# rimelabs/lambda-labs_distributed-training-guide

Measured on AMD Instinct MI355X. Metric: tokens/sec/GPU (causal-LM pretrain) at 1/2/4/8 MI355X; FSDP peak-mem, higher is better.
Workload: dtype bf16; 1 GPU; model=meta-llama/Meta-Llama-3-8B, global_batch=16, seq_len=1024, parallelism=dp1-single

## Files before the change

csrc/kernels/flash_attn.hip:

```cpp
#include "flash_attn_plan.h"
#include "rope_common.h"

#include <ATen/hip/HIPGeneratorImpl.h>
#include <ATen/hip/PhiloxUtils.cuh>
#include <ATen/core/DistributionsHelper.h>

#include <climits>
#include <cstdlib>
#include <type_traits>

#include <cmath>

namespace dtg {

namespace fa {

typedef __attribute__((address_space(3))) i16x4 lds_i16x4;

constexpr float kLog2e = 1.4426950408889634f;
constexpr float kLn2 = 0.6931471805599453f;
constexpr float kRescaleThreshold = 8.f;

template <int W>
__device__ __forceinline__ int off(int row, int ch) {
// ... 176 lines not shown
    for (int j = 0; j < 2; ++j) {
      uint32_t w[4];
#pragma unroll
      for (int u = 0; u < 2; ++u) {
        const int base = 4 * (2 * j + u);
        w[2 * u + 0] = (uint32_t)f2bf(acc[d][base + 0] * scale) | ((uint32_t)f2bf(acc[d][base + 1] * scale) << 16);
        w[2 * u + 1] = (uint32_t)f2bf(acc[d][base + 2] * scale) | ((uint32_t)f2bf(acc[d][base + 3] * scale) << 16);
      }
#pragma unroll
      for (int x = 0; x < 2; ++x) {
        const auto r = __builtin_amdgcn_permlane32_swap(w[x], w[2 + x], false, false);
        w[x] = r[0];
        w[2 + x] = r[1];
      }
      if (ok) *reinterpret_cast<uint4*>(row + 32 * d + 16 * j + 8 * h) = make_uint4(w[0], w[1], w[2], w[3]);
    }
  }
}

struct KeyRange {
  int start, len, off;
};
__device__ __forceinline__ KeyRange key_range(const int* kstart, const int* klen, int seq, int s0, int seqlen) {
  if (kstart == nullptr) return KeyRange{s0, seqlen, 0};
  const int n = klen[seq];
  return KeyRange{kstart[seq], n, n - seqlen};
}

struct FwdParams {
  const uint16_t *q, *k, *v;
// ... 198 lines not shown
  const float* lse;
  float* delta;
  uint16_t *dq, *dk, *dv;
  int64_t sdq, sdk, sdv;
  const int* cu;
  int64_t T;
  int hq, hkv;
  float scale, c2;
  const int *kstart, *klen;
  int window;
  float *dk_part, *dv_part;
  int nsplit;
  DropCfg drop;
  const float *rope_cos, *rope_sin;
  const int64_t* rope_pos;
};

template <int ND>
__device__ __forceinline__ void rope_inv_rows(f32x16* acc, const float* cos_t, const float* sin_t, int64_t p) {
  constexpr int HT = ND / 2;
  constexpr int HALF = 16 * ND;
  const int h = (threadIdx.x & 63) >> 5;
  const float* cp = cos_t + p * HALF;
  const float* sp = sin_t + p * HALF;
#pragma unroll
  for (int d = 0; d < HT; ++d) {
#pragma unroll
    for (int g = 0; g < 4; ++g) {
      const int i = 32 * d + 8 * g + 4 * h;
      const float4 c = *reinterpret_cast<const float4*>(cp + i);
      const float4 sn = *reinterpret_cast<const float4*>(sp + i);
      const float cc[4] = {c.x, c.y, c.z, c.w}, ss[4] = {sn.x, sn.y, sn.z, sn.w};
#pragma unroll
      for (int e = 0; e < 4; ++e) {
        const int r = 4 * g + e;
        const float x1 = acc[d][r], x2 = acc[d + HT][r];
        acc[d][r] = x1 * cc[e] + x2 * ss[e];
        acc[d + HT][r] = x2 * cc[e] - x1 * ss[e];
      }
    }
  }
}

template <int D, bool CAUSAL, int OCC, bool WIN = false, bool DROP = false>
__global__ __launch_bounds__(256, OCC) void bwd_dq_kernel(BwdParams P) {
  [[maybe_unused]] const DropCfg dcfg = DROP ? resolve_drop(P.drop) : P.drop;
  constexpr int RB = 2 * D;
  constexpr int TILE = kDqBK * RB;
  constexpr int NC = D / 16;
  constexpr int ND = D / 32;
  extern __shared__ __attribute__((aligned(16))) char smem[];

  const int seq = blockIdx.y, head = grid_head(blockIdx.x, P.hq, P.hkv);
  const int s0 = P.cu[seq];
  const int seqlen = P.cu[seq + 1] - s0;
  const int qb = CAUSAL ? (gridDim.z - 1 - blockIdx.z) : blockIdx.z;
  const int q0 = qb * kDqBQ;
  if (q0 >= seqlen) return;
  const KeyRange kr = key_range(P.kstart, P.klen, seq, s0, seqlen);
// ... 152 lines not shown
      char* nb = smem + (1 - B) * 2 * TILE;
      sk.store(nb);
      sv.store(nb + TILE);
    }
    __syncthreads();
  };
  int t = t_begin;
  for (; t + 1 < ntiles; t += 2) {
    tile_step(t, std::integral_constant<int, 0>{});
    tile_step(t + 1, std::integral_constant<int, 1>{});
  }
  if (t < ntiles) tile_step(t, std::integral_constant<int, 0>{});

  if (P.rope_cos != nullptr) rope_inv_rows<ND>(acc, P.rope_cos, P.rope_sin, P.rope_pos[s0 + min(qrow, seqlen - 1)]);
  store_rows_wide<ND>(acc, P.scale, P.dq + (int64_t)(s0 + min(qrow, seqlen - 1)) * P.sdq + (int64_t)head * D, qok);
}

template <int D, bool CAUSAL, int PF, bool WIN = false, int QB = kKvBQ, bool DROP = false>
__global__ __launch_bounds__(256, D == 128 ? 1 : 2) void bwd_dkdv_kernel(BwdParams P) {
  [[maybe_unused]] const DropCfg dcfg = DROP ? resolve_drop(P.drop) : P.drop;
  static_assert(QB == 32 || QB == 64, "query rows per item");
  constexpr int RB = 2 * D;
  constexpr int NC = D / 16;
  constexpr int ND = D / 32;
  constexpr int SLICE = QB * RB;
  extern __shared__ __attribute__((aligned(16))) char smem[];
  char* qd = smem;
  float* rowc = reinterpret_cast<float*>(qd + 4 * SLICE);

  const int seq = blockIdx.y, kvh = blockIdx.x;
  const int s0 = P.cu[seq];
  const int seqlen = P.cu[seq + 1] - s0;
  const KeyRange kr = key_range(P.kstart, P.klen, seq, s0, seqlen);
// ... 269 lines not shown
      float* pv = P.dv_part + o;
#pragma unroll
      for (int d = 0; d < ND; ++d) {
#pragma unroll
        for (int g = 0; g < 4; ++g) {
          *reinterpret_cast<f32x4*>(pk + 32 * d + 8 * g) = f32x4{dk[d][4 * g], dk[d][4 * g + 1], dk[d][4 * g + 2], dk[d][4 * g + 3]};
          *reinterpret_cast<f32x4*>(pv + 32 * d + 8 * g) = f32x4{dv[d][4 * g], dv[d][4 * g + 1], dv[d][4 * g + 2], dv[d][4 * g + 3]};
        }
      }
    }
    return;
  }
  if (P.rope_cos != nullptr) rope_inv_rows<ND>(dk, P.rope_cos, P.rope_sin, P.rope_pos[krow]);
  store_rows_wide<ND>(dk, P.scale, P.dk + krow * P.sdk + (int64_t)kvh * D, key < klen);
  store_rows_wide<ND>(dv, 1.f, P.dv + krow * P.sdv + (int64_t)kvh * D, key < klen);
}

template <int D>
__global__ __launch_bounds__(256) void bwd_kv_combine_kernel(const float* __restrict__ dk_part,
                                                             const float* __restrict__ dv_part, int nsplit,
                                                             int64_t T, int hkv, float scale, uint16_t* __restrict__ dk,
                                                             int64_t sdk, uint16_t* __restrict__ dv, int64_t sdv) {
  constexpr int V = D / 8;
  const int64_t i = (int64_t)blockIdx.x * blockDim.x + threadIdx.x;
  const int64_t rows = T * hkv;
  if (i >= rows * V) return;
  const int64_t row = i / V;
  const int c = (int)(i % V) * 8;
  const int64_t t = row / hkv;
  const int hh = (int)(row % hkv);
// ... 8 lines not shown
    for (int j = 0; j < 4; ++j) {
      a[j] += k0[j];
      a[4 + j] += k1[j];
      b[j] += v0[j];
      b[4 + j] += v1[j];
    }
  }
#pragma unroll
  for (int j = 0; j < 8; ++j) a[j] *= scale;
  store8(dk + t * sdk + (int64_t)hh * D + c, a);
  store8(dv + t * sdv + (int64_t)hh * D + c, b);
}

}

static int env_int(const char* name, int dflt) {
  const char* e = std::getenv(name);
  return (e != nullptr && e[0] != 0) ? std::atoi(e) : dflt;
}
static fa::Tuning& tuning() {
  static fa::Tuning t{std::max(0, env_int("DTG_FA_KV_SPLIT", 0)), env_int("DTG_FA_KV_QB", 64) == 32 ? 32 : 64,
                      env_int("DTG_FA_OCC", 1) == 2 ? 2 : 1, env_int("DTG_FA_KV_PF", 1) == 2 ? 2 : 1};
  return t;
}
[[maybe_unused]] static const bool kTuningLoaded = (tuning(), true);

std::vector<int64_t> flash_attn_tuning(const at::Tensor& , int64_t kv_split, int64_t kv_qb) {
  fa::Tuning& t = tuning();
  std::vector<int64_t> old{t.kv_split, t.kv_qb};
  if (kv_split >= 0) t.kv_split = (int)kv_split;
// ... 2 lines not shown
  return old;
}

template <typename Params>
static void launch(void (*kernel)(Params), const fa::Plan& pl, size_t lds, hipStream_t st, const Params& P) {
  TORCH_INTERNAL_ASSERT(lds == pl.lds, "flash_attn: launch plan and instantiation disagree");
  if (lds > 65536)
    C10_HIP_CHECK(hipFuncSetAttribute((const void*)kernel, hipFuncAttributeMaxDynamicSharedMemorySize, (int)lds));
  hipLaunchKernelGGL(kernel, dim3(pl.grid.x, pl.grid.y, pl.grid.z), dim3(256), lds, st, P);
  DTG_LAUNCH_CHECK();
}
template <int D, bool C, bool WIN = false, bool DROP = false>
static void fwd_launch(const fa::FwdPlan& pl, const fa::FwdParams& P, hipStream_t st) {
  launch(fa::fwd_kernel<D, C, WIN, DROP>, pl, fa::fwd_lds_bytes(D), st, P);
}
template <int D, bool C, int OCC, bool WIN = false, bool DROP = false>
static void dq_launch(const fa::DqPlan& pl, const fa::BwdParams& P, hipStream_t st) {
  TORCH_INTERNAL_ASSERT(pl.occ == OCC);
  launch(fa::bwd_dq_kernel<D, C, OCC, WIN, DROP>, pl, fa::dq_lds_bytes(D), st, P);
}
template <int D, bool C, int PF, bool WIN = false, int QB = fa::kKvBQ, bool DROP = false>
static void kv_launch(const fa::KvPlan& pl, const fa::BwdParams& P, hipStream_t st) {
  TORCH_INTERNAL_ASSERT(pl.pf == PF && pl.qb == QB);
  launch(fa::bwd_dkdv_kernel<D, C, PF, WIN, QB, DROP>, pl, fa::kv_lds_bytes(D, QB), st, P);
}

template <int D>
static void launch_fwd(const fa::FwdPlan& pl, const fa::FwdParams& P, hipStream_t st) {
  if (pl.var == fa::Variant::DROP)
    pl.causal ? fwd_launch<D, true, false, true>(pl, P, st) : fwd_launch<D, false, false, true>(pl, P, st);
  else if (pl.var == fa::Variant::WIN) fwd_launch<D, true, true>(pl, P, st);
  else pl.causal ? fwd_launch<D, true>(pl, P, st) : fwd_launch<D, false>(pl, P, st);
}
template <int D>
static void launch_bwd_dq(const fa::DqPlan& pl, const fa::BwdParams& P, hipStream_t st) {
  constexpr int kOcc = D == 64 ? 2 : 1;
  if (pl.var == fa::Variant::DROP)
    pl.causal ? dq_launch<D, true, kOcc, false, true>(pl, P, st) : dq_launch<D, false, kOcc, false, true>(pl, P, st);
  else if (pl.var == fa::Variant::WIN) dq_launch<D, true, kOcc, true>(pl, P, st);
  else if (pl.occ == 2) pl.causal ? dq_launch<D, true, 2>(pl, P, st) : dq_launch<D, false, 2>(pl, P, st);
  else pl.causal ? dq_launch<D, true, kOcc>(pl, P, st) : dq_launch<D, false, kOcc>(pl, P, st);
}
template <int D>
static void launch_bwd_dkdv(const fa::KvPlan& pl, fa::BwdParams P, hipStream_t st, const at::TensorOptions& opts) {
  at::Tensor dk_part, dv_part;
  P.nsplit = pl.nsplit;
  if (pl.nsplit > 1) {
    dk_part = at::empty({pl.nsplit, P.T, P.hkv, D}, opts.dtype(at::kFloat));
    dv_part = at::empty({pl.nsplit, P.T, P.hkv, D}, opts.dtype(at::kFloat));
    P.dk_part = dk_part.data_ptr<float>();
    P.dv_part = dv_part.data_ptr<float>();
  }
  if (pl.var == fa::Variant::DROP)
    pl.causal ? kv_launch<D, true, 1, false, 64, true>(pl, P, st) : kv_launch<D, false, 1, false, 64, true>(pl, P, st);
  else if (pl.var == fa::Variant::WIN) kv_launch<D, true, 1, true>(pl, P, st);
  else if (pl.pf == 2) pl.causal ? kv_launch<D, true, 2>(pl, P, st) : kv_launch<D, false, 2>(pl, P, st);
  else if (pl.qb == 64)
    pl.causal ? kv_launch<D, true, 1, false, 64>(pl, P, st) : kv_launch<D, false, 1, false, 64>(pl, P, st);
  else pl.causal ? kv_launch<D, true, 1>(pl, P, st) : kv_launch<D, false, 1>(pl, P, st);
  if (pl.nsplit > 1) {
    const int64_t nv = P.T * P.hkv * (D / 8);
    fa::bwd_kv_combine_kernel<D><<<(nv + 255) / 256, 256, 0, st>>>(P.dk_part, P.dv_part, pl.nsplit, P.T, P.hkv, P.scale,
                                                                  P.dk, P.sdk, P.dv, P.sdv);
    DTG_LAUNCH_CHECK();
    if (P.rope_cos != nullptr) rope_rows_launch(P.dk, P.sdk, P.hkv, D, P.rope_cos, P.rope_sin, P.rope_pos, P.T, true, st);
  }
}

struct AttnOpts {
  const at::Tensor *k_start = nullptr, *k_len = nullptr;
  int64_t max_seqlen_k = -1;
  int64_t window = 0;
  const fa::DropCfg* drop = nullptr;
  const at::Tensor *rope_cos = nullptr, *rope_sin = nullptr, *rope_pos = nullptr;
  at::Tensor* stamps = nullptr;
};

static void check_qkv(const at::Tensor& t, const char* name, int64_t heads, int64_t d) {
  DTG_CHECK_CUDA_BF16(t);
  DTG_CHECK(t.dim() == 3 && t.size(1) == heads && t.size(2) == d && t.stride(2) == 1 &&
                t.stride(1) == d && t.stride(0) % 8 == 0,
            name, " must be [T, H, D] with contiguous heads and 16-B aligned token stride");
}

static void check_inputs(const at::Tensor& q, const at::Tensor& k, const at::Tensor& v, const at::Tensor& cu_seqlens) {
  const int64_t D = q.size(2);
  check_qkv(q, "q", q.size(1), D);
  check_qkv(k, "k", k.size(1), D);
  check_qkv(v, "v", k.size(1), D);
  DTG_CHECK(D == 64 || D == 128, "flash_attn: head_dim must be 64 or 128");
// ... 81 lines not shown
  fa::BwdParams P{bf16_ptr(q), bf16_ptr(k), bf16_ptr(v), bf16_ptr(dout), bf16_ptr(o), q.stride(0), k.stride(0),
                  v.stride(0), lse.data_ptr<float>(), delta.data_ptr<float>(), bf16_mut(dq), bf16_mut(dk),
                  bf16_mut(dv), dq.stride(0), dk.stride(0), dv.stride(0), cu_seqlens.data_ptr<int>(), T, (int)hq,
                  (int)hkv, (float)scale, (float)(scale * fa::kLog2e), nullptr, nullptr, 0};
  const fa::Call c = checked_call(q, hkv, nseq, max_seqlen, causal, op, &P.kstart, &P.klen);
  P.window = fa::window_eff(c);
  if (op.rope_cos != nullptr) {
    P.rope_cos = op.rope_cos->data_ptr<float>();
    P.rope_sin = op.rope_sin->data_ptr<float>();
    P.rope_pos = op.rope_pos->data_ptr<int64_t>();
  }
  if (const char* why = fa::conflict(c)) DTG_CHECK(false, why);
  if (op.drop != nullptr) P.drop = *op.drop;
  const fa::DqPlan dqp = fa::plan_dq(c, tuning());
  const fa::KvPlan kvp = fa::plan_kv(c, tuning());
  D == 128 ? launch_bwd_dq<128>(dqp, P, stream()) : launch_bwd_dq<64>(dqp, P, stream());
  D == 128 ? launch_bwd_dkdv<128>(kvp, P, stream(), q.options()) : launch_bwd_dkdv<64>(kvp, P, stream(), q.options());
}

static std::tuple<at::Tensor, at::Tensor, at::Tensor> flash_attn_bwd_alloc(
    const at::Tensor& dout, const at::Tensor& q, const at::Tensor& k, const at::Tensor& v, const at::Tensor& o,
    const at::Tensor& lse, const at::Tensor& cu_seqlens, int64_t max_seqlen, double scale, bool causal,
    const AttnOpts& op) {
  auto dq = at::empty(q.sizes(), q.options());
  auto dk = op.k_start != nullptr ? at::zeros(k.sizes(), k.options()) : at::empty(k.sizes(), k.options());
  auto dv = op.k_start != nullptr ? at::zeros(v.sizes(), v.options()) : at::empty(v.sizes(), v.options());
  flash_attn_bwd_impl(dout, q, k, v, o, lse, cu_seqlens, max_seqlen, scale, causal, dq, dk, dv, op);
  return {dq, dk, dv};
}

static at::Tensor flash_attn_bwd_fused(const char* name, const at::Tensor& dout, const at::Tensor& qkv, int64_t nq,
                                       int64_t nkv, int64_t D, const at::Tensor& o, const at::Tensor& lse,
                                       const at::Tensor& cu_seqlens, int64_t max_seqlen, double scale, bool causal,
                                       const AttnOpts& op) {
  rope::check_qkv(qkv, nq + 2 * nkv, D, name);
  const int64_t T = qkv.size(0);
  DTG_CHECK(qkv.size(1) == (nq + 2 * nkv) * D, name, ": qkv must be [T, (nq + 2 nkv) * D]");
  if (op.rope_cos != nullptr) {
    rope::check_tables(*op.rope_cos, *op.rope_sin, D, name);
    rope::check_pos(*op.rope_pos, T, name);
  }
  auto dqkv = at::empty({T, (nq + 2 * nkv) * D}, qkv.options());
  auto view3 = [&](const at::Tensor& t, int64_t h0, int64_t nh) {
    return t.as_strided({T, nh, D}, {t.stride(0), D, 1}, t.storage_offset() + h0 * D);
  };
  flash_attn_bwd_impl(dout, view3(qkv, 0, nq), view3(qkv, nq, nkv), view3(qkv, nq + nkv, nkv), o, lse, cu_seqlens,
                      max_seqlen, scale, causal, view3(dqkv, 0, nq), view3(dqkv, nq, nkv), view3(dqkv, nq + nkv, nkv), op);
  return dqkv;
}

std::tuple<at::Tensor, at::Tensor, at::Tensor> flash_attn_bwd(
    const at::Tensor& dout, const at::Tensor& q, const at::Tensor& k, const at::Tensor& v, const at::Tensor& o,
    const at::Tensor& lse, const at::Tensor& cu_seqlens, int64_t max_seqlen, double scale, bool causal, int64_t window) {
  return flash_attn_bwd_alloc(dout, q, k, v, o, lse, cu_seqlens, max_seqlen, scale, causal, {.window = window});
}

at::Tensor flash_attn_bwd_qkv(const at::Tensor& dout, const at::Tensor& qkv, int64_t nq, int64_t nkv, int64_t head_dim,
                              const at::Tensor& o, const at::Tensor& lse, const at::Tensor& cu_seqlens,
                              int64_t max_seqlen, double scale, bool causal, int64_t window) {
  return flash_attn_bwd_fused("flash_attn_bwd_qkv", dout, qkv, nq, nkv, head_dim, o, lse, cu_seqlens, max_seqlen, scale,
                              causal, {.window = window});
}

at::Tensor flash_attn_bwd_qkv_rope(const at::Tensor& dout, const at::Tensor& qkv, int64_t nq, int64_t nkv, int64_t head_dim,
                                   const at::Tensor& o, const at::Tensor& lse, const at::Tensor& cu_seqlens,
                                   int64_t max_seqlen, double scale, bool causal, const at::Tensor& cos_t,
                                   const at::Tensor& sin_t, const at::Tensor& pos, int64_t window) {
  return flash_attn_bwd_fused("flash_attn_bwd_qkv_rope", dout, qkv, nq, nkv, head_dim, o, lse, cu_seqlens, max_seqlen,
                              scale, causal, {.window = window, .rope_cos = &cos_t, .rope_sin = &sin_t, .rope_pos = &pos});
}

std::tuple<at::Tensor, at::Tensor> flash_attn_varlen_fwd(
    const at::Tensor& q, const at::Tensor& k, const at::Tensor& v, const at::Tensor& cu_seqlens_q,
    const at::Tensor& k_start, const at::Tensor& k_len, int64_t max_seqlen_q,
    int64_t , double scale, bool causal) {
  return flash_attn_fwd_impl(q, k, v, cu_seqlens_q, max_seqlen_q, scale, causal, {.k_start = &k_start, .k_len = &k_len});
}

std::tuple<at::Tensor, at::Tensor, at::Tensor> flash_attn_varlen_bwd(
    const at::Tensor& dout, const at::Tensor& q, const at::Tensor& k, const at::Tensor& v, const at::Tensor& o,
    const at::Tensor& lse, const at::Tensor& cu_seqlens_q, const at::Tensor& k_start, const at::Tensor& k_len,
    int64_t max_seqlen_q, int64_t max_seqlen_k, double scale, bool causal) {
  return flash_attn_bwd_alloc(dout, q, k, v, o, lse, cu_seqlens_q, max_seqlen_q, scale, causal,
                              {.k_start = &k_start, .k_len = &k_len, .max_seqlen_k = max_seqlen_k});
// ... 58 lines not shown
  return out;
}

TORCH_LIBRARY_IMPL(dtg, CUDA, m) {
  m.impl("flash_attn_fwd_drop", &flash_attn_fwd_drop);
  m.impl("flash_attn_bwd_drop", &flash_attn_bwd_drop);
  m.impl("flash_attn_bwd_qkv_drop", &flash_attn_bwd_qkv_drop);
  m.impl("philox_rng", &philox_rng);
  m.impl("flash_attn_varlen_fwd", &flash_attn_varlen_fwd);
  m.impl("flash_attn_varlen_bwd", &flash_attn_varlen_bwd);
  m.impl("flash_attn_fwd", &flash_attn_fwd);
  m.impl("flash_attn_fwd_stamped", &flash_attn_fwd_stamped);
  m.impl("flash_attn_bwd", &flash_attn_bwd);
  m.impl("flash_attn_bwd_qkv", &flash_attn_bwd_qkv);
  m.impl("flash_attn_bwd_qkv_rope", &flash_attn_bwd_qkv_rope);
  m.impl("flash_attn_tuning", &flash_attn_tuning);
}

}
```

csrc/kernels/flash_attn_plan.h:

```cpp
#pragma once

#include <algorithm>
#include <cstddef>
#include <cstdint>

namespace dtg {
namespace fa {

constexpr int kFwdBQ = 128;
constexpr int kFwdBK = 64;
constexpr int kDqBQ = 128;
constexpr int kDqBK = 64;
constexpr int kKvBK = 128;
constexpr int kKvBQ = 32;

constexpr size_t fwd_lds_bytes(int D) { return 4 * (size_t)kFwdBK * D * 2; }
constexpr size_t dq_lds_bytes(int D) { return 4 * (size_t)kDqBK * D * 2 + kDqBQ * 4; }
constexpr size_t kv_lds_bytes(int D, int qb) { return 4 * (size_t)qb * D * 2 + 2 * 2 * qb * 4; }

struct Tuning {
  int kv_split, kv_qb, dq_occ, kv_pf;
};
struct Call {
  int D;
// ... 42 lines not shown
}

inline KvPlan plan_kv(const Call& c, const Tuning& t) {
  const Variant var = variant(c);
  const int pf = var == Variant::PLAIN && !c.key_ranges ? t.kv_pf : 1;
  const int qb = c.drop || (t.kv_qb != 32 && window_eff(c) == 0 && t.kv_pf == 1) ? 64 : 32;
  const unsigned nkb = nblocks(c.max_seqlen_k, kKvBK);
  const int64_t wgs = (int64_t)c.hkv * c.nseq * nkb;
  int nsplit = 1;
  if (t.kv_split > 0) nsplit = std::min(8, t.kv_split);
  else if (wgs > 0 && wgs < 512) nsplit = (int)std::min<int64_t>(4, (512 + wgs - 1) / wgs);
  if (c.key_ranges || window_eff(c) != 0 || (c.drop ? 1 : t.kv_pf) != 1) nsplit = 1;
  return {{var, c.causal, {(unsigned)c.hkv, (unsigned)c.nseq, nkb * nsplit}, kv_lds_bytes(c.D, qb)}, pf, qb, nsplit};
}

}
}
```

lambda-labs_distributed-training-guide_amd/models/llama.py:

```python
from __future__ import annotations

import dataclasses
import weakref
from typing import Optional

import torch
import torch.distributed as dist
import torch.nn as nn

from .. import ops
from ..parallel import async_tp, tp_comm
from .config import LlamaConfig


@dataclasses.dataclass
class CausalLMOutput:
    loss: Optional[torch.Tensor] = None
    logits: Optional[torch.Tensor] = None


class Weight(nn.Module):

    _dtg_param_holder = True

# ... 59 lines not shown
            k = qkv[:, self.nq * d:(self.nq + self.nkv) * d].reshape(T, self.nkv, d)
            v = qkv[:, (self.nq + self.nkv) * d:].reshape(T, self.nkv, d)
            return cp_attention(q, k, v, rc.cp_group, rc.rows, ranges=rc.cp_ranges).reshape(T, self.nq * d)
        if rc.sp_group is not None:
            from ..parallel.ulysses import ulysses_attention

            qkv = ops.qk_norm_rope(qkv, wq, wk, self.eps, self.nq, self.nkv, d)
            return ulysses_attention(qkv, self.nq, self.nkv, d, rc.sp_group, rc.rows, rc.cu_seqlens,
                                     rc.max_seqlen, rc.cos, rc.sin, rc.pos)
        qkv = ops.qk_norm_rope(qkv, wq, wk, self.eps, self.nq, self.nkv, d, rc.cos, rc.sin, rc.pos,
                               grad_inplace=True)
        return ops.attention(qkv, self.nq, self.nkv, d, rc.cu_seqlens, rc.max_seqlen, window=self.window)

    def forward(self, x, rc: RunCtx, out=None):
        b = getattr(self.qkv_proj, "bias", None)
        qkv = ops.linear(x, self.qkv_proj.weight, None if b is None else b.view(-1))
        if self.qk_norm:
            return ops.linear(self._forward_qk_norm(qkv, rc), self.o_proj.weight, out=out)
        if rc.cp_group is not None:
            from ..parallel.context_parallel import cp_attention

            T, d = qkv.shape[0], self.d
            qkv = ops.rope(qkv, rc.cos, rc.sin, rc.pos, self.nq + self.nkv, d)
            q = qkv[:, :self.nq * d].reshape(T, self.nq, d)
            k = qkv[:, self.nq * d:(self.nq + self.nkv) * d].reshape(T, self.nkv, d)
            v = qkv[:, (self.nq + self.nkv) * d:].reshape(T, self.nkv, d)
            o = cp_attention(q, k, v, rc.cp_group, rc.rows, ranges=rc.cp_ranges).reshape(T, self.nq * d)
        elif rc.sp_group is not None:
            from ..parallel.ulysses import ulysses_attention

# ... 295 lines not shown
```

lambda-labs_distributed-training-guide_amd/ops/__init__.py:

```python
from . import _schema
from . import _cpu
from . import _native

_native.load()
if not _native.LOADED:
    _schema.LIB.impl("adamw_cpu_", lambda p, g, m, v, lr, b1, b2, eps, wd, step, gs: _cpu.adamw_(
        p, None, g, m, v, lr, b1, b2, eps, wd, step, gs), "CPU")

from .functional import (
    add_rms_norm,
    attention,
    check_sample_scalar,
    decode_attention,
    decode_attention_multi,
    dropout_add_layer_norm,
    embedding,
    fused_linear_cross_entropy,
    gelu_mlp,
    kv_cache_append,
    layer_norm,
    linear,
    qk_norm_rope,
    quantize_fp8_rows,
    rms_norm,
    rope,
    rope_tables,
    sample_logits,
    skinny_linear,
    skinny_linear_fp8,
    swiglu,
    swiglu_mlp,
    vocab_parallel_fused_linear_cross_entropy,
)
from .grad_routing import route_param_grad
from .adamw import adamw_step

import contextlib as _contextlib
# ... 3 lines not shown

@_contextlib.contextmanager
def fa_tuning(device="cuda", kv_split: int = -1, kv_qb: int = -1):
    like = _torch.empty(0, device=device)
    old = _torch.ops.dtg.flash_attn_tuning(like, kv_split, kv_qb)
    try:
        yield
    finally:
        _torch.ops.dtg.flash_attn_tuning(like, old[0], old[1])

__all__ = [
    "add_rms_norm", "attention", "rope", "embedding", "fused_linear_cross_entropy", "linear", "rms_norm",
    "rope_tables", "swiglu", "swiglu_mlp", "vocab_parallel_fused_linear_cross_entropy", "route_param_grad", "adamw_step",
    "fa_tuning", "layer_norm", "dropout_add_layer_norm", "gelu_mlp", "qk_norm_rope", "kv_cache_append", "decode_attention",
    "sample_logits", "skinny_linear", "skinny_linear_fp8", "quantize_fp8_rows", "decode_attention_multi",
]
```

lambda-labs_distributed-training-guide_amd/ops/_cpu.py:

```python
import math

import torch
import torch.nn.functional as F

from ._schema import LIB

_LOG2E = 1.4426950408889634


def rmsnorm_fwd(x, w, eps):
    xf = x.float()
    rstd = torch.rsqrt(xf.pow(2).mean(-1) + eps)
    n = (xf * rstd[:, None]).to(x.dtype)
    y = (w.float() * n.float()).to(x.dtype)
    return y, rstd


def add_rmsnorm_fwd(x, res, w, eps):
    h = (x.float() + res.float()).to(x.dtype)
    y, rstd = rmsnorm_fwd(h, w, eps)
    return y, h, rstd


def rmsnorm_bwd(dy, x, w, rstd, dres):
# ... 674 lines not shown
    q, k, v = _qkv_heads(qkv, nq, nkv, head_dim)
    dq, dk, dv = flash_attn_bwd(dout, q, k, v, o, lse, cu_seqlens, max_seqlen, scale, causal, window)
    return torch.cat([dq.reshape(T, -1), dk.reshape(T, -1), dv.reshape(T, -1)], dim=1)


def flash_attn_bwd_qkv_rope(dout, qkv, nq, nkv, head_dim, o, lse, cu_seqlens, max_seqlen, scale, causal, cos, sin,
                            pos, window=0):
    T = qkv.shape[0]
    q, k, v = _qkv_heads(qkv, nq, nkv, head_dim)
    dq, dk, dv = _flash_attn_bwd_f32(dout, q, k, v, o, lse, cu_seqlens, max_seqlen, scale, causal, window)
    dqkv = torch.cat([dq.reshape(T, -1), dk.reshape(T, -1), dv.reshape(T, -1)], dim=1)
    rope_(dqkv, cos, sin, pos, nq + nkv, head_dim, True)
    return dqkv.to(qkv.dtype)


def swiglu_bwd_t(dh, gu):
    if not (gu.dim() == 2 and gu.stride(1) == 1 and gu.stride(0) % 8 == 0 and gu.shape[1] % 16 == 0):
        raise RuntimeError("dtg: swiglu_bwd_t: the pre-activation must be [T, 2 * I] with unit inner stride, "
                           "16-byte aligned rows and I % 8 == 0")
    if not (dh.dim() == 2 and dh.shape[0] == gu.shape[0] and dh.shape[1] == gu.shape[1] // 2):
        raise RuntimeError("dtg: swiglu_bwd_t: shape mismatch")
    dgu = swiglu_bwd(dh, gu)
    return dgu, dgu.t().contiguous(), swiglu_fwd(gu).t().contiguous()


def transpose2d(x):
    return x.t().contiguous()


def transpose_mats_(x, out, mats, mats_host, ntiles):
# ... 84 lines not shown
def flash_attn_tuning(like, kv_split, kv_qb):
    old = list(_TUNING)
    if kv_split >= 0:
        _TUNING[0] = int(kv_split)
    if kv_qb >= 0:
        _TUNING[1] = int(kv_qb)
    return old


for _name, _fn in list(globals().items()):
    if _name in (
        "rmsnorm_fwd", "add_rmsnorm_fwd", "rmsnorm_bwd", "rope_", "swiglu_fwd", "swiglu_bwd",
        "ce_fwd_bwd_", "ce_stats", "ce_grad_", "adamw_", "adamw_t_", "grad_sumsq_", "flash_attn_fwd", "flash_attn_bwd",
        "flash_attn_bwd_qkv", "transpose2d", "transpose_mats_", "swiglu_bwd_t", "embedding_bwd_", "flash_attn_varlen_fwd",
        "flash_attn_varlen_bwd", "flash_attn_fwd_drop", "flash_attn_bwd_drop", "flash_attn_bwd_qkv_drop", "philox_rng",
        "flash_attn_bwd_qkv_rope", "flash_attn_tuning", "layernorm_fwd", "dropout_add_layernorm_fwd", "layernorm_bwd",
        "gelu_fwd", "gelu_bwd", "gelu_bwd_t", "qk_norm_rope_fwd_", "qk_norm_rope_bwd_", "kv_cache_append_", "decode_attn",
        "sample_logits", "skinny_linear", "skinny_linear_fp8", "decode_attn_multi",
        "kv_cache_append_fp8_", "decode_attn_fp8",
    ):
        LIB.impl(_name, _fn, "CPU")
```

lambda-labs_distributed-training-guide_amd/ops/_schema.py:

```python
import torch

LIB = torch.library.Library("dtg", "DEF")

_DEFS = [
    "rmsnorm_fwd(Tensor x, Tensor w, float eps) -> (Tensor, Tensor)",
    "add_rmsnorm_fwd(Tensor x, Tensor residual, Tensor w, float eps) -> (Tensor, Tensor, Tensor)",
    "rmsnorm_bwd(Tensor dy, Tensor x, Tensor w, Tensor rstd, Tensor? dres) -> (Tensor, Tensor)",
    "layernorm_fwd(Tensor x, Tensor w, Tensor b, float eps) -> (Tensor, Tensor, Tensor)",
    "dropout_add_layernorm_fwd(Tensor x, Tensor residual, Tensor w, Tensor b, float eps, float p, Tensor? rng) "
    "-> (Tensor, Tensor, Tensor, Tensor)",
    "layernorm_bwd(Tensor dy, Tensor h, Tensor w, Tensor mean, Tensor rstd, Tensor? dres, float p, Tensor? rng) "
    "-> (Tensor, Tensor, Tensor, Tensor)",
    "gelu_fwd(Tensor x) -> Tensor",
    "gelu_bwd(Tensor dh, Tensor x) -> Tensor",
    "gelu_bwd_t(Tensor dh, Tensor x) -> (Tensor, Tensor, Tensor)",
    "rope_(Tensor(a!) qkv, Tensor cos, Tensor sin, Tensor pos, int nheads, int head_dim, bool inverse) -> ()",
    "qk_norm_rope_fwd_(Tensor(a!) qkv, Tensor wq, Tensor wk, Tensor cos, Tensor sin, Tensor pos, int nq, int nkv, "
    "int head_dim, float eps) -> (Tensor, Tensor)",
    "qk_norm_rope_bwd_(Tensor(a!) dqkv, Tensor xqk, Tensor rstd, Tensor wq, Tensor wk, Tensor cos, Tensor sin, "
    "Tensor pos, int nq, int nkv, int head_dim) -> (Tensor, Tensor)",
    "kv_cache_append_(Tensor(a!) qkv, Tensor(b!) k_cache, Tensor(c!) v_cache, Tensor cos, Tensor sin, Tensor pos, "
    "Tensor rows, int nq, int nkv, int head_dim) -> ()",
    "decode_attn(Tensor qkv, Tensor k_cache, Tensor v_cache, Tensor rows, Tensor lens, int nq, int nkv, int head_dim, "
    "float scale, int max_len, int window=0, int splits=0) -> Tensor",
# ... 17 lines not shown
    "adamw_t_(Tensor(a!) p, Tensor(b!)? master, Tensor g, Tensor(c!) m, Tensor(d!) v, Tensor(e!) pt, Tensor mats, "
    "int ntiles, float lr, float beta1, float beta2, float eps, float wd, int step, float grad_scale, "
    "Tensor? hyper=None, int tile_cols=64, Tensor? gscale=None) -> ()",
    "grad_sumsq_(Tensor g, Tensor(a!) acc, int slot) -> ()",
    "adamw_cpu_(Tensor(a!) p, Tensor g, Tensor(b!) m, Tensor(c!) v, float lr, float beta1, float beta2, "
    "float eps, float wd, int step, float grad_scale) -> ()",
    "flash_attn_fwd(Tensor q, Tensor k, Tensor v, Tensor cu_seqlens, int max_seqlen, float scale, bool causal, "
    "int window=0) -> (Tensor, Tensor)",
    "flash_attn_bwd(Tensor dout, Tensor q, Tensor k, Tensor v, Tensor o, Tensor lse, Tensor cu_seqlens, "
    "int max_seqlen, float scale, bool causal, int window=0) -> (Tensor, Tensor, Tensor)",
    "flash_attn_bwd_qkv(Tensor dout, Tensor qkv, int nq, int nkv, int head_dim, Tensor o, Tensor lse, "
    "Tensor cu_seqlens, int max_seqlen, float scale, bool causal, int window=0) -> Tensor",
    "flash_attn_bwd_qkv_rope(Tensor dout, Tensor qkv, int nq, int nkv, int head_dim, Tensor o, Tensor lse, "
    "Tensor cu_seqlens, int max_seqlen, float scale, bool causal, Tensor cos, Tensor sin, Tensor pos, "
    "int window=0) -> Tensor",
    "flash_attn_fwd_drop(Tensor q, Tensor k, Tensor v, Tensor cu_seqlens, int max_seqlen, float scale, bool causal, "
    "float p, Tensor rng) -> (Tensor, Tensor)",
    "flash_attn_bwd_drop(Tensor dout, Tensor q, Tensor k, Tensor v, Tensor o, Tensor lse, Tensor cu_seqlens, "
    "int max_seqlen, float scale, bool causal, float p, Tensor rng) -> (Tensor, Tensor, Tensor)",
    "flash_attn_bwd_qkv_drop(Tensor dout, Tensor qkv, int nq, int nkv, int head_dim, Tensor o, Tensor lse, "
    "Tensor cu_seqlens, int max_seqlen, float scale, bool causal, float p, Tensor rng) -> Tensor",
    "philox_rng(Tensor like, int increment) -> Tensor",
    "transpose2d(Tensor x) -> Tensor",
    "transpose_mats_(Tensor x, Tensor(a!) out, Tensor mats, Tensor mats_host, int ntiles) -> ()",
    "embedding_bwd_(Tensor(a!) out, Tensor ids, Tensor dy) -> ()",
    "flash_attn_varlen_fwd(Tensor q, Tensor k, Tensor v, Tensor cu_seqlens_q, Tensor k_start, Tensor k_len, "
    "int max_seqlen_q, int max_seqlen_k, float scale, bool causal) -> (Tensor, Tensor)",
    "flash_attn_varlen_bwd(Tensor dout, Tensor q, Tensor k, Tensor v, Tensor o, Tensor lse, Tensor cu_seqlens_q, "
    "Tensor k_start, Tensor k_len, int max_seqlen_q, int max_seqlen_k, float scale, bool causal) "
    "-> (Tensor, Tensor, Tensor)",
# ... 8 lines not shown
```

lambda-labs_distributed-training-guide_amd/ops/functional.py:

```python
import math
import os

import torch
import torch.distributed as dist
import torch.nn.functional as F

from . import grad_routing as _gr
from ._cpu import SKINNY_MAX_M
from .grad_routing import route_embedding_grad, route_param_grad, route_weight_grad_mm

ops = torch.ops.dtg


_LINEAR_BWD = os.environ.get("DTG_LINEAR_BWD", "tn")
_TN_MIN_TOKENS = 4096


def _tn_ok(*ts):
    return all(t.is_cuda and t.dtype == torch.bfloat16 and t.shape[0] % 8 == 0 and t.shape[1] % 8 == 0
               and t.stride(1) == 1 for t in ts)


def _wt(w):
    ref = getattr(w, "_dtg_wt", None)
# ... 211 lines not shown

    @staticmethod
    def backward(ctx, do):
        qkv, o, lse, cu, cos, sin, pos = ctx.saved_tensors
        max_seqlen, nq, nkv, d, scale, causal, rope, window = ctx.meta
        T = qkv.shape[0]
        if rope and _FA_ROPE_FUSED:
            dqkv = ops.flash_attn_bwd_qkv_rope(do.contiguous().view(T, nq, d), qkv, nq, nkv, d, o, lse, cu, max_seqlen,
                                               scale, causal, cos, sin, pos, window)
        else:
            dqkv = ops.flash_attn_bwd_qkv(do.contiguous().view(T, nq, d), qkv, nq, nkv, d, o, lse, cu, max_seqlen,
                                          scale, causal, window)
            if rope:
                ops.rope_(dqkv, cos, sin, pos, nq + nkv, d, True)
        return dqkv, None, None, None, None, None, None, None, None, None, None, None, None


class _AttentionQKVDrop(torch.autograd.Function):

    @staticmethod
    def forward(ctx, qkv, cu_seqlens, max_seqlen, nq, nkv, head_dim, scale, causal, p, rng):
        T = qkv.shape[0]
        d = head_dim
        q, k, v = _qkv_head_views(qkv, nq, nkv, d)
        o, lse = ops.flash_attn_fwd_drop(q, k, v, cu_seqlens, max_seqlen, scale, causal, p, rng)
        ctx.save_for_backward(qkv, o, lse, cu_seqlens, rng)
        ctx.meta = (max_seqlen, nq, nkv, d, scale, causal, p)
        return o.view(T, nq * d)

    @staticmethod
# ... 695 lines not shown
```

Before: 27740 tokens/s (whole job).

## Fuse QKV projection with attention and emit transposed dQKV from backward kernels

Adds a combined QKV-projection + flash-attention autograd function whose backward asks the flash-attention dq and dkdv kernels to also write a transposed copy of dQKV, scattered column-wise. That copy then feeds the weight-gradient matmul directly. The aim is to drop the separate transpose pass and the extra layout traffic when computing dW in TN layout. The cost is strided, uncoalesced 2-byte column stores from the attention kernels, plus one extra [3D*heads, T] buffer.

```diff
diff --git a/csrc/kernels/flash_attn.hip b/csrc/kernels/flash_attn.hip
--- a/csrc/kernels/flash_attn.hip
+++ b/csrc/kernels/flash_attn.hip
@@ -214,6 +214,20 @@
         w[2 + x] = r[1];
       }
       if (ok) *reinterpret_cast<uint4*>(row + 32 * d + 16 * j + 8 * h) = make_uint4(w[0], w[1], w[2], w[3]);
+    }
+  }
+}
+
+template <int ND>
+__device__ __forceinline__ void store_cols_t(const f32x16* acc, float scale, uint16_t* col0, int64_t T, bool ok) {
+  if (!ok) return;
+  const int h = (threadIdx.x & 63) >> 5;
+#pragma unroll
+  for (int d = 0; d < ND; ++d) {
+#pragma unroll
+    for (int g = 0; g < 4; ++g) {
+#pragma unroll
+      for (int e = 0; e < 4; ++e) col0[(int64_t)(32 * d + 8 * g + 4 * h + e) * T] = f2bf(acc[d][4 * g + e] * scale);
     }
   }
 }
@@ -442,6 +456,7 @@
   DropCfg drop;
   const float *rope_cos, *rope_sin;
   const int64_t* rope_pos;
+  uint16_t *dq_t, *dk_t, *dv_t;
 };
 
 template <int ND>
@@ -470,7 +485,7 @@
   }
 }
 
-template <int D, bool CAUSAL, int OCC, bool WIN = false, bool DROP = false>
+template <int D, bool CAUSAL, int OCC, bool WIN = false, bool DROP = false, bool TR = false>
 __global__ __launch_bounds__(256, OCC) void bwd_dq_kernel(BwdParams P) {
   [[maybe_unused]] const DropCfg dcfg = DROP ? resolve_drop(P.drop) : P.drop;
   constexpr int RB = 2 * D;
@@ -653,9 +668,10 @@
 
   if (P.rope_cos != nullptr) rope_inv_rows<ND>(acc, P.rope_cos, P.rope_sin, P.rope_pos[s0 + min(qrow, seqlen - 1)]);
   store_rows_wide<ND>(acc, P.scale, P.dq + (int64_t)(s0 + min(qrow, seqlen - 1)) * P.sdq + (int64_t)head * D, qok);
-}
-
-template <int D, bool CAUSAL, int PF, bool WIN = false, int QB = kKvBQ, bool DROP = false>
+  if constexpr (TR) store_cols_t<ND>(acc, P.scale, P.dq_t + (int64_t)head * D * P.T + t_row, P.T, qok);
+}
+
+template <int D, bool CAUSAL, int PF, bool WIN = false, int QB = kKvBQ, bool DROP = false, bool TR = false>
 __global__ __launch_bounds__(256, D == 128 ? 1 : 2) void bwd_dkdv_kernel(BwdParams P) {
   [[maybe_unused]] const DropCfg dcfg = DROP ? resolve_drop(P.drop) : P.drop;
   static_assert(QB == 32 || QB == 64, "query rows per item");
@@ -955,6 +971,10 @@
   if (P.rope_cos != nullptr) rope_inv_rows<ND>(dk, P.rope_cos, P.rope_sin, P.rope_pos[krow]);
   store_rows_wide<ND>(dk, P.scale, P.dk + krow * P.sdk + (int64_t)kvh * D, key < klen);
   store_rows_wide<ND>(dv, 1.f, P.dv + krow * P.sdv + (int64_t)kvh * D, key < klen);
+  if constexpr (TR) {
+    store_cols_t<ND>(dk, P.scale, P.dk_t + (int64_t)kvh * D * P.T + krow, P.T, key < klen);
+    store_cols_t<ND>(dv, 1.f, P.dv_t + (int64_t)kvh * D * P.T + krow, P.T, key < klen);
+  }
 }
 
 template <int D>
@@ -993,6 +1013,8 @@
 
 }
 
+at::Tensor transpose2d(const at::Tensor& x);
+
 static int env_int(const char* name, int dflt) {
   const char* e = std::getenv(name);
   return (e != nullptr && e[0] != 0) ? std::atoi(e) : dflt;
@@ -1025,15 +1047,15 @@
 static void fwd_launch(const fa::FwdPlan& pl, const fa::FwdParams& P, hipStream_t st) {
   launch(fa::fwd_kernel<D, C, WIN, DROP>, pl, fa::fwd_lds_bytes(D), st, P);
 }
-template <int D, bool C, int OCC, bool WIN = false, bool DROP = false>
+template <int D, bool C, int OCC, bool WIN = false, bool DROP = false, bool TR = false>
 static void dq_launch(const fa::DqPlan& pl, const fa::BwdParams& P, hipStream_t st) {
-  TORCH_INTERNAL_ASSERT(pl.occ == OCC);
-  launch(fa::bwd_dq_kernel<D, C, OCC, WIN, DROP>, pl, fa::dq_lds_bytes(D), st, P);
-}
-template <int D, bool C, int PF, bool WIN = false, int QB = fa::kKvBQ, bool DROP = false>
+  TORCH_INTERNAL_ASSERT(pl.occ == OCC && TR == (P.dq_t != nullptr));
+  launch(fa::bwd_dq_kernel<D, C, OCC, WIN, DROP, TR>, pl, fa::dq_lds_bytes(D), st, P);
+}
+template <int D, bool C, int PF, bool WIN = false, int QB = fa::kKvBQ, bool DROP = false, bool TR = false>
 static void kv_launch(const fa::KvPlan& pl, const fa::BwdParams& P, hipStream_t st) {
-  TORCH_INTERNAL_ASSERT(pl.pf == PF && pl.qb == QB);
-  launch(fa::bwd_dkdv_kernel<D, C, PF, WIN, QB, DROP>, pl, fa::kv_lds_bytes(D, QB), st, P);
+  TORCH_INTERNAL_ASSERT(pl.pf == PF && pl.qb == QB && TR == (P.dk_t != nullptr));
+  launch(fa::bwd_dkdv_kernel<D, C, PF, WIN, QB, DROP, TR>, pl, fa::kv_lds_bytes(D, QB), st, P);
 }
 
 template <int D>
@@ -1046,7 +1068,11 @@
 template <int D>
 static void launch_bwd_dq(const fa::DqPlan& pl, const fa::BwdParams& P, hipStream_t st) {
   constexpr int kOcc = D == 64 ? 2 : 1;
-  if (pl.var == fa::Variant::DROP)
+  if (P.dq_t != nullptr) {
+    TORCH_INTERNAL_ASSERT(fa::dq_emits_t(pl, D));
+    pl.causal ? dq_launch<D, true, kOcc, false, false, true>(pl, P, st)
+              : dq_launch<D, false, kOcc, false, false, true>(pl, P, st);
+  } else if (pl.var == fa::Variant::DROP)
     pl.causal ? dq_launch<D, true, kOcc, false, true>(pl, P, st) : dq_launch<D, false, kOcc, false, true>(pl, P, st);
   else if (pl.var == fa::Variant::WIN) dq_launch<D, true, kOcc, true>(pl, P, st);
   else if (pl.occ == 2) pl.causal ? dq_launch<D, true, 2>(pl, P, st) : dq_launch<D, false, 2>(pl, P, st);
@@ -1062,7 +1088,11 @@
     P.dk_part = dk_part.data_ptr<float>();
     P.dv_part = dv_part.data_ptr<float>();
   }
-  if (pl.var == fa::Variant::DROP)
+  if (P.dk_t != nullptr) {
+    TORCH_INTERNAL_ASSERT(fa::kv_emits_t(pl));
+    pl.causal ? kv_launch<D, true, 1, false, 64, false, true>(pl, P, st)
+              : kv_launch<D, false, 1, false, 64, false, true>(pl, P, st);
+  } else if (pl.var == fa::Variant::DROP)
     pl.causal ? kv_launch<D, true, 1, false, 64, true>(pl, P, st) : kv_launch<D, false, 1, false, 64, true>(pl, P, st);
   else if (pl.var == fa::Variant::WIN) kv_launch<D, true, 1, true>(pl, P, st);
   else if (pl.pf == 2) pl.causal ? kv_launch<D, true, 2>(pl, P, st) : kv_launch<D, false, 2>(pl, P, st);
@@ -1085,6 +1115,8 @@
   const fa::DropCfg* drop = nullptr;
   const at::Tensor *rope_cos = nullptr, *rope_sin = nullptr, *rope_pos = nullptr;
   at::Tensor* stamps = nullptr;
+  const at::Tensor* dqkv_t = nullptr;
+  bool* dqkv_t_written = nullptr;
 };
 
 static void check_qkv(const at::Tensor& t, const char* name, int64_t heads, int64_t d) {
@@ -1196,6 +1228,12 @@
   if (op.drop != nullptr) P.drop = *op.drop;
   const fa::DqPlan dqp = fa::plan_dq(c, tuning());
   const fa::KvPlan kvp = fa::plan_kv(c, tuning());
+  if (op.dqkv_t != nullptr && op.k_start == nullptr && fa::dq_emits_t(dqp, (int)D) && fa::kv_emits_t(kvp)) {
+    P.dq_t = bf16_mut(*op.dqkv_t);
+    P.dk_t = P.dq_t + hq * D * T;
+    P.dv_t = P.dk_t + hkv * D * T;
+    *op.dqkv_t_written = true;
+  }
   D == 128 ? launch_bwd_dq<128>(dqp, P, stream()) : launch_bwd_dq<64>(dqp, P, stream());
   D == 128 ? launch_bwd_dkdv<128>(kvp, P, stream(), q.options()) : launch_bwd_dkdv<64>(kvp, P, stream(), q.options());
 }
@@ -1214,7 +1252,7 @@
 static at::Tensor flash_attn_bwd_fused(const char* name, const at::Tensor& dout, const at::Tensor& qkv, int64_t nq,
                                        int64_t nkv, int64_t D, const at::Tensor& o, const at::Tensor& lse,
                                        const at::Tensor& cu_seqlens, int64_t max_seqlen, double scale, bool causal,
-                                       const AttnOpts& op) {
+                                       AttnOpts op, at::Tensor* dqkv_t = nullptr) {
   rope::check_qkv(qkv, nq + 2 * nkv, D, name);
   const int64_t T = qkv.size(0);
   DTG_CHECK(qkv.size(1) == (nq + 2 * nkv) * D, name, ": qkv must be [T, (nq + 2 nkv) * D]");
@@ -1223,11 +1261,18 @@
     rope::check_pos(*op.rope_pos, T, name);
   }
   auto dqkv = at::empty({T, (nq + 2 * nkv) * D}, qkv.options());
+  bool t_written = false;
+  if (dqkv_t != nullptr) {
+    *dqkv_t = at::empty({(nq + 2 * nkv) * D, T}, qkv.options());
+    op.dqkv_t = dqkv_t;
+    op.dqkv_t_written = &t_written;
+  }
   auto view3 = [&](const at::Tensor& t, int64_t h0, int64_t nh) {
     return t.as_strided({T, nh, D}, {t.stride(0), D, 1}, t.storage_offset() + h0 * D);
   };
   flash_attn_bwd_impl(dout, view3(qkv, 0, nq), view3(qkv, nq, nkv), view3(qkv, nq + nkv, nkv), o, lse, cu_seqlens,
                       max_seqlen, scale, causal, view3(dqkv, 0, nq), view3(dqkv, nq, nkv), view3(dqkv, nq + nkv, nkv), op);
+  if (dqkv_t != nullptr && !t_written) *dqkv_t = transpose2d(dqkv);
   return dqkv;
 }
 
@@ -1250,6 +1295,26 @@
                                    const at::Tensor& sin_t, const at::Tensor& pos, int64_t window) {
   return flash_attn_bwd_fused("flash_attn_bwd_qkv_rope", dout, qkv, nq, nkv, head_dim, o, lse, cu_seqlens, max_seqlen,
                               scale, causal, {.window = window, .rope_cos = &cos_t, .rope_sin = &sin_t, .rope_pos = &pos});
+}
+
+std::tuple<at::Tensor, at::Tensor> flash_attn_bwd_qkv_t(
+    const at::Tensor& dout, const at::Tensor& qkv, int64_t nq, int64_t nkv, int64_t head_dim, const at::Tensor& o,
+    const at::Tensor& lse, const at::Tensor& cu_seqlens, int64_t max_seqlen, double scale, bool causal,
+    const c10::optional<at::Tensor>& cos_t, const c10::optional<at::Tensor>& sin_t,
+    const c10::optional<at::Tensor>& pos, int64_t window) {
+  const bool rope = cos_t.has_value();
+  DTG_CHECK(rope == sin_t.has_value() && rope == pos.has_value(), "flash_attn_bwd_qkv_t: cos, sin and pos go together");
+  DTG_CHECK(qkv.dim() == 2 && qkv.size(0) % 8 == 0, "flash_attn_bwd_qkv_t: the token count must be a multiple of 8");
+  AttnOpts op{.window = window};
+  if (rope) {
+    op.rope_cos = &*cos_t;
+    op.rope_sin = &*sin_t;
+    op.rope_pos = &*pos;
+  }
+  at::Tensor dqkv_t;
+  auto dqkv = flash_attn_bwd_fused("flash_attn_bwd_qkv_t", dout, qkv, nq, nkv, head_dim, o, lse, cu_seqlens, max_seqlen,
+                                   scale, causal, op, &dqkv_t);
+  return {dqkv, dqkv_t};
 }
 
 std::tuple<at::Tensor, at::Tensor> flash_attn_varlen_fwd(
@@ -1338,6 +1403,7 @@
   m.impl("flash_attn_bwd", &flash_attn_bwd);
   m.impl("flash_attn_bwd_qkv", &flash_attn_bwd_qkv);
   m.impl("flash_attn_bwd_qkv_rope", &flash_attn_bwd_qkv_rope);
+  m.impl("flash_attn_bwd_qkv_t", &flash_attn_bwd_qkv_t);
   m.impl("flash_attn_tuning", &flash_attn_tuning);
 }
 
diff --git a/csrc/kernels/flash_attn_plan.h b/csrc/kernels/flash_attn_plan.h
--- a/csrc/kernels/flash_attn_plan.h
+++ b/csrc/kernels/flash_attn_plan.h
@@ -80,5 +80,8 @@
   return {{var, c.causal, {(unsigned)c.hkv, (unsigned)c.nseq, nkb * nsplit}, kv_lds_bytes(c.D, qb)}, pf, qb, nsplit};
 }
 
+inline bool dq_emits_t(const DqPlan& p, int D) { return p.var == Variant::PLAIN && p.occ == (D == 64 ? 2 : 1); }
+inline bool kv_emits_t(const KvPlan& p) { return p.var == Variant::PLAIN && p.pf == 1 && p.qb == 64 && p.nsplit <= 1; }
+
 }
 }
diff --git a/lambda-labs_distributed-training-guide_amd/models/llama.py b/lambda-labs_distributed-training-guide_amd/models/llama.py
--- a/lambda-labs_distributed-training-guide_amd/models/llama.py
+++ b/lambda-labs_distributed-training-guide_amd/models/llama.py
@@ -97,6 +97,10 @@
 
     def forward(self, x, rc: RunCtx, out=None):
         b = getattr(self.qkv_proj, "bias", None)
+        if b is None and not self.qk_norm and rc.cp_group is None and rc.sp_group is None:
+            o = ops.qkv_attention(x, self.qkv_proj.weight, self.nq, self.nkv, self.d, rc.cu_seqlens, rc.max_seqlen,
+                                  rc.cos, rc.sin, rc.pos, window=self.window)
+            return ops.linear(o, self.o_proj.weight, out=out)
         qkv = ops.linear(x, self.qkv_proj.weight, None if b is None else b.view(-1))
         if self.qk_norm:
             return ops.linear(self._forward_qk_norm(qkv, rc), self.o_proj.weight, out=out)
diff --git a/lambda-labs_distributed-training-guide_amd/ops/__init__.py b/lambda-labs_distributed-training-guide_amd/ops/__init__.py
--- a/lambda-labs_distributed-training-guide_amd/ops/__init__.py
+++ b/lambda-labs_distributed-training-guide_amd/ops/__init__.py
@@ -21,6 +21,7 @@
     layer_norm,
     linear,
     qk_norm_rope,
+    qkv_attention,
     quantize_fp8_rows,
     rms_norm,
     rope,
@@ -54,4 +55,5 @@
     "rope_tables", "swiglu", "swiglu_mlp", "vocab_parallel_fused_linear_cross_entropy", "route_param_grad", "adamw_step",
     "fa_tuning", "layer_norm", "dropout_add_layer_norm", "gelu_mlp", "qk_norm_rope", "kv_cache_append", "decode_attention",
     "sample_logits", "skinny_linear", "skinny_linear_fp8", "quantize_fp8_rows", "decode_attention_multi",
+    "qkv_attention",
 ]
diff --git a/lambda-labs_distributed-training-guide_amd/ops/_cpu.py b/lambda-labs_distributed-training-guide_amd/ops/_cpu.py
--- a/lambda-labs_distributed-training-guide_amd/ops/_cpu.py
+++ b/lambda-labs_distributed-training-guide_amd/ops/_cpu.py
@@ -712,6 +712,20 @@
     return dqkv.to(qkv.dtype)
 
 
+def flash_attn_bwd_qkv_t(dout, qkv, nq, nkv, head_dim, o, lse, cu_seqlens, max_seqlen, scale, causal, cos, sin, pos,
+                         window=0):
+    if (cos is None) != (sin is None) or (cos is None) != (pos is None):
+        raise RuntimeError("dtg: flash_attn_bwd_qkv_t: cos, sin and pos go together")
+    if qkv.shape[0] % 8:
+        raise RuntimeError("dtg: flash_attn_bwd_qkv_t: the token count must be a multiple of 8")
+    if cos is None:
+        dqkv = flash_attn_bwd_qkv(dout, qkv, nq, nkv, head_dim, o, lse, cu_seqlens, max_seqlen, scale, causal, window)
+    else:
+        dqkv = flash_attn_bwd_qkv_rope(dout, qkv, nq, nkv, head_dim, o, lse, cu_seqlens, max_seqlen, scale, causal, cos,
+                                       sin, pos, window)
+    return dqkv, dqkv.t().contiguous()
+
+
 def swiglu_bwd_t(dh, gu):
     if not (gu.dim() == 2 and gu.stride(1) == 1 and gu.stride(0) % 8 == 0 and gu.shape[1] % 16 == 0):
         raise RuntimeError("dtg: swiglu_bwd_t: the pre-activation must be [T, 2 * I] with unit inner stride, "
@@ -826,7 +840,7 @@
         "ce_fwd_bwd_", "ce_stats", "ce_grad_", "adamw_", "adamw_t_", "grad_sumsq_", "flash_attn_fwd", "flash_attn_bwd",
         "flash_attn_bwd_qkv", "transpose2d", "transpose_mats_", "swiglu_bwd_t", "embedding_bwd_", "flash_attn_varlen_fwd",
         "flash_attn_varlen_bwd", "flash_attn_fwd_drop", "flash_attn_bwd_drop", "flash_attn_bwd_qkv_drop", "philox_rng",
-        "flash_attn_bwd_qkv_rope", "flash_attn_tuning", "layernorm_fwd", "dropout_add_layernorm_fwd", "layernorm_bwd",
+        "flash_attn_bwd_qkv_rope", "flash_attn_bwd_qkv_t", "flash_attn_tuning", "layernorm_fwd", "dropout_add_layernorm_fwd", "layernorm_bwd",
         "gelu_fwd", "gelu_bwd", "gelu_bwd_t", "qk_norm_rope_fwd_", "qk_norm_rope_bwd_", "kv_cache_append_", "decode_attn",
         "sample_logits", "skinny_linear", "skinny_linear_fp8", "decode_attn_multi",
         "kv_cache_append_fp8_", "decode_attn_fp8",
diff --git a/lambda-labs_distributed-training-guide_amd/ops/_schema.py b/lambda-labs_distributed-training-guide_amd/ops/_schema.py
--- a/lambda-labs_distributed-training-guide_amd/ops/_schema.py
+++ b/lambda-labs_distributed-training-guide_amd/ops/_schema.py
@@ -55,6 +55,9 @@
     "flash_attn_bwd_qkv_rope(Tensor dout, Tensor qkv, int nq, int nkv, int head_dim, Tensor o, Tensor lse, "
     "Tensor cu_seqlens, int max_seqlen, float scale, bool causal, Tensor cos, Tensor sin, Tensor pos, "
     "int window=0) -> Tensor",
+    "flash_attn_bwd_qkv_t(Tensor dout, Tensor qkv, int nq, int nkv, int head_dim, Tensor o, Tensor lse, "
+    "Tensor cu_seqlens, int max_seqlen, float scale, bool causal, Tensor? cos, Tensor? sin, Tensor? pos, "
+    "int window=0) -> (Tensor, Tensor)",
     "flash_attn_fwd_drop(Tensor q, Tensor k, Tensor v, Tensor cu_seqlens, int max_seqlen, float scale, bool causal, "
     "float p, Tensor rng) -> (Tensor, Tensor)",
     "flash_attn_bwd_drop(Tensor dout, Tensor q, Tensor k, Tensor v, Tensor o, Tensor lse, Tensor cu_seqlens, "
diff --git a/lambda-labs_distributed-training-guide_amd/ops/functional.py b/lambda-labs_distributed-training-guide_amd/ops/functional.py
--- a/lambda-labs_distributed-training-guide_amd/ops/functional.py
+++ b/lambda-labs_distributed-training-guide_amd/ops/functional.py
@@ -249,6 +249,63 @@
             if rope:
                 ops.rope_(dqkv, cos, sin, pos, nq + nkv, d, True)
         return dqkv, None, None, None, None, None, None, None, None, None, None, None, None
+
+
+_FUSED_T = os.environ.get("DTG_FUSED_T", "1") == "1"
+
+
+class _QKVAttention(torch.autograd.Function):
+
+    @staticmethod
+    def forward(ctx, x, w, cos, sin, pos, cu_seqlens, max_seqlen, nq, nkv, head_dim, scale, causal, rope, window):
+        T, d = x.shape[0], head_dim
+        qkv = torch.mm(x, w.t())
+        if rope:
+            ops.rope_(qkv, cos, sin, pos, nq + nkv, d, False)
+        q, k, v = _qkv_head_views(qkv, nq, nkv, d)
+        o, lse = ops.flash_attn_fwd(q, k, v, cu_seqlens, max_seqlen, scale, causal, window)
+        ctx.save_for_backward(x, w, qkv, o, lse, cu_seqlens, cos, sin, pos)
+        ctx.meta = (max_seqlen, nq, nkv, d, scale, causal, rope, window)
+        return o.view(T, nq * d)
+
+    @staticmethod
+    def backward(ctx, do):
+        x, w, qkv, o, lse, cu, cos, sin, pos = ctx.saved_tensors
+        max_seqlen, nq, nkv, d, scale, causal, rope, window = ctx.meta
+        T = qkv.shape[0]
+        dx_tn, dw_tn = _bwd_layout(x, w)
+        do = do.contiguous().view(T, nq, d)
+        fused_rope = rope and _FA_ROPE_FUSED
+        dqkv_t = None
+        if _FUSED_T and dw_tn and ctx.needs_input_grad[1] and _tn_ok(qkv) and (fused_rope or not rope):
+            r = (cos, sin, pos) if fused_rope else (None, None, None)
+            dqkv, dqkv_t = ops.flash_attn_bwd_qkv_t(do, qkv, nq, nkv, d, o, lse, cu, max_seqlen, scale, causal, *r, window)
+        elif fused_rope:
+            dqkv = ops.flash_attn_bwd_qkv_rope(do, qkv, nq, nkv, d, o, lse, cu, max_seqlen, scale, causal, cos, sin, pos,
+                                               window)
+        else:
+            dqkv = ops.flash_attn_bwd_qkv(do, qkv, nq, nkv, d, o, lse, cu, max_seqlen, scale, causal, window)
+            if rope:
+                ops.rope_(dqkv, cos, sin, pos, nq + nkv, d, True)
+        del qkv, o, lse, do
+        dx = _dx_mm(dqkv, w, dx_tn) if ctx.needs_input_grad[0] else None
+        dw = _dw_mm(w, dqkv, x, dw_tn, dy_t=dqkv_t) if ctx.needs_input_grad[1] else None
+        del dqkv_t
+        return (dx, dw) + (None,) * 12
+
+
+def qkv_attention(x, w, nq, nkv, head_dim, cu_seqlens, max_seqlen, cos=None, sin=None, pos=None, causal=True,
+                  scale=None, window=0):
+    if x.is_cuda and head_dim not in FA_HEAD_DIMS:
+        return attention(linear(x, w), nq, nkv, head_dim, cu_seqlens, max_seqlen, cos, sin, pos, causal, scale, window)
+    if scale is None:
+        scale = 1.0 / math.sqrt(head_dim)
+    rope = cos is not None
+    if not rope:
+        cos = sin = torch.empty(0, device=x.device)
+        pos = torch.empty(0, dtype=torch.long, device=x.device)
+    return _QKVAttention.apply(x, w, cos, sin, pos, cu_seqlens, int(max_seqlen), nq, nkv, head_dim, float(scale), causal,
+                               rope, int(window or 0))
 
 
 class _AttentionQKVDrop(torch.autograd.Function):
```

Measured after the change: 27770 tokens/s (whole job) (median of 5 runs). About the same (+0.1%).
